# AegisIK/DistMLIP

Measured on NVIDIA H100. Metric: atoms/sec (energy+forces) CHGNet a-Si r_cut=5A, higher is better.
Workload: dtype f32

## Files before the change

### distmlip_b200/csrc/engine.cu

```cuda
#include <dlfcn.h>
#include <nccl.h>

#include <cmath>
#include <condition_variable>
#include <mutex>
#include <thread>
#include <cstring>
#include <map>
#include <new>
#include <set>
#include <string>
#include <vector>

#include <algorithm>
#include <array>

#include "atomic_virial.cuh"
#include "graph.cuh"
#include "kernels.cuh"
#include "mace_state.cuh"
#include "tn_state.cuh"

namespace b2m {

// ... 207 lines not shown
  for (int n = 0; n < N; n++)
    for (int k = 0; k < K; k++) {
      const size_t off = ((size_t)(k / 4) * (N / 8) + n / 8) * 32 + (n % 8) * 4 + (k % 4);
      const float x = raw[(size_t)n * K + k];
      const float h = tf32_hi_host(x);
      o[off] = h;
      o[(size_t)N * Kpad + off] = x - h;
    }
  return o;
}

static std::vector<float> permute_k8(const std::vector<float>& raw, int N, int K) {
  std::vector<float> o(raw.size());
  for (int n = 0; n < N; n++)
    for (int k = 0; k < K; k++) {
      const int q = k % 8;
      o[(size_t)n * K + k] = raw[(size_t)n * K + (k - q) + (q < 4 ? 2 * q : 2 * (q - 4) + 1)];
    }
  return o;
}

static std::vector<float> second_layer_can(const std::vector<float>& raw128x64, bool transposed) {
  std::vector<float> out;
  for (int br = 0; br < 2; br++) {
    std::vector<float> blk(raw128x64.begin() + (size_t)br * 4096, raw128x64.begin() + (size_t)(br + 1) * 4096);
    if (transposed) blk = transpose(blk, 64, 64);
    const auto c = canon_split(permute_k8(blk, 64, 64), 64, 64, 64);
    out.insert(out.end(), c.begin(), c.end());
  }
  return out;
}
static std::vector<float> line_reverse_can(const std::vector<float>& raw128x64) {
  return canon_split(permute_k8(transpose(raw128x64, 128, 64), 64, 128), 64, 128, 128);
}
static std::vector<float> radial_can(const std::vector<float>& M, const std::vector<float>& Wab) {
  auto k8 = [](const std::vector<float>& w, int row0) {
    std::vector<float> o(64 * 8);
    for (int n = 0; n < 64; n++)
      for (int k = 0; k < 8; k++) o[(size_t)n * 8 + k] = w[(size_t)(row0 + n) * NR + k];
    return canon_split(permute_k8(o, 64, 8), 64, 8, 8);
  };
  std::vector<float> out;
  for (const auto& c : {k8(M, 0), k8(M, 64), k8(Wab, 0)}) out.insert(out.end(), c.begin(), c.end());
  for (int j = 0; j < 128; j++) out.push_back(M[(size_t)j * NR + 8]);
  for (int c = 0; c < 64; c++) out.push_back(Wab[(size_t)c * NR + 8]);
  B2M_REQUIRE(out.size() == ATOM_RAD, B2M_ERR_INVALID, "atom-conv radial block size");
  return out;
}

static TcW pack_tc(Packer& P, const std::vector<float>& W, int K, int N, int kmax = 128) {
  TcW w;
  w.K = K, w.N = N;
  for (int k0 = 0; k0 < K;) {
    const int kc = K - k0 >= kmax ? kmax : 64;
    for (int n0 = 0; n0 < N;) {
      const int nc = kc == 64 && N - n0 >= 128 ? 128 : 64;
      std::vector<float> raw((size_t)nc * kc);
      for (int n = 0; n < nc; n++)
        for (int k = 0; k < kc; k++) raw[(size_t)n * kc + k] = W[(size_t)(k0 + k) * N + n0 + n];
      w.blk.push_back({k0, kc, n0, nc, P.add(canon_split(raw, nc, kc, kc))});
      n0 += nc;
    }
    k0 += kc;
  }
  return w;
}
static void pack_tc2(Packer& P, const std::vector<float>& W, int K, int N, TcW& fwd, TcW& rev, int rev_kmax = 128) {
  fwd = pack_tc(P, W, K, N);
  rev = pack_tc(P, transpose(W, K, N), N, K, rev_kmax);
}
static void tc_mm(b2m_engine* e, const float* A, int lda, const TcW& W, float* out, int ldc, int M, bool accum,
                  const float* bias = nullptr, const float* R = nullptr, int ldr = 0, int epi = 0, float* Cpre = nullptr,
                  const float* Pre = nullptr, int ldp = 0) {
  B2M_REQUIRE(epi != 1 || W.blk.back().k0 == 0, B2M_ERR_INVALID, "row GEMM: SiLU epilogue over several K chunks");
  for (const TcW::Blk& b : W.blk) {
    const bool first = b.k0 == 0, last = b.k0 + b.kc == W.K;
    launch_gemm_wg(e->st, A + b.k0, lda, e->wbuf.p + b.off, out + b.n0, ldc, M, b.nc, b.kc,
                   first && bias ? bias + b.n0 : nullptr, first && R ? R + b.n0 : nullptr, ldr, accum || !first,
                   epi == 2 && !last ? 0 : epi, Cpre ? Cpre + b.n0 : nullptr, epi == 2 && last ? Pre + b.n0 : nullptr,
                   ldp, e->num_sms);
  }
}

static void finalize_weights(b2m_engine* e) {
  const int nb = e->desc.n_blocks;
  for (auto& kv : e->host_w) {
    const std::string& k = kv.first;
    bool bad = k.find("atom_graph_layers") != std::string::npos &&
               (k.find("edge_update_func") != std::string::npos || k.find("weight_func") != std::string::npos);
    bad = bad || (k.find("bond_graph_layers") != std::string::npos && k.find("weight_func") != std::string::npos);
    bad = bad || k.find("state_embedding") != std::string::npos || k.find("normalization") != std::string::npos;
    B2M_REQUIRE(!bad, B2M_ERR_INVALID,
                "unsupported CHGNet option (bond_update_hidden_dims / layer_bond_weights / state / norm): " + k);
  }
  e->consumed.clear();
  Packer P;
  std::map<std::string, size_t> off;
  auto put = [&](const std::string& name, const std::vector<float>& v) { off[name] = P.add(v); };
  auto linear = [&](const std::vector<float>& w, int out, int in, TcW& fwd, TcW& rev) {
    pack_tc2(P, transpose(w, out, in), in, out, fwd, rev);
  };

  const auto& f2 = W(e, "bond_expansion.frequencies", {NR});
  const auto& f3 = W(e, "threebody_bond_expansion.frequencies", {NR});
  const auto& fa = W(e, "angle_expansion.frequencies", {5});
  for (int k = 0; k < NR; k++) {
    e->rp2.freq[k] = f2[k];
    e->rp3.freq[k] = f3[k];
  }
  e->rp2.rc = (float)e->desc.cutoff;
  e->rp3.rc = (float)e->desc.three_body_cutoff;
  e->rp2.norm = (float)std::sqrt(2.0 / e->desc.cutoff);
  e->rp3.norm = (float)std::sqrt(2.0 / e->desc.three_body_cutoff);
  e->rp2.p = e->rp3.p = e->desc.cutoff_exponent;
  put("fa", fa);
  put("emb", W(e, "atom_embedding.weight", {e->desc.n_elem, D}));
  const auto& Wbe = W(e, "bond_embedding.layers.0.weight", {D, NR});
  put("Wbe", Wbe);
  put("Wae", W(e, "angle_embedding.layers.0.weight", {D, NF}));
  const auto& Wabw = W(e, "atom_bond_weights.weight", {D, NR});
  put("W3bw", W(e, "threebody_bond_weights.weight", {D, NR}));

  e->aw.resize(nb);
  for (int l = 0; l < nb; l++) {
    const std::string p = "atom_graph_layers." + std::to_string(l) + ".conv_layer.";
    const auto W1 = vcat(W(e, p + "node_update_func.layers.layers.0.weight", {D, 3 * D}),
                         W(e, p + "node_update_func.gates.layers.0.weight", {D, 3 * D}));
    const auto b1 = vcat(W(e, p + "node_update_func.layers.layers.0.bias", {D}),
                         W(e, p + "node_update_func.gates.layers.0.bias", {D}));
    const auto W1s = cols(W1, 128, 192, 0), W1e = cols(W1, 128, 192, 64), W1t = cols(W1, 128, 192, 128);
    const auto W2 = vcat(W(e, p + "node_update_func.layers.layers.1.weight", {D, D}),
                         W(e, p + "node_update_func.gates.layers.1.weight", {D, D}));
    const auto b2 = vcat(W(e, p + "node_update_func.layers.layers.1.bias", {D}),
                         W(e, p + "node_update_func.gates.layers.1.bias", {D}));
    const auto& Wout = W(e, p + "node_out_func.weight", {D, D});
    std::vector<float> M(128 * 9);
    for (int j = 0; j < 128; j++)
      for (int k = 0; k < 9; k++) {
        double s = 0;
        for (int c = 0; c < 64; c++) s += (double)W1e[(size_t)j * 64 + c] * (double)Wbe[(size_t)c * 9 + k];
        M[j * 9 + k] = (float)s;
      }
    const std::string q = "a" + std::to_string(l) + ".";
    AtomLayerW& w = e->aw[l];
    linear(W1s, 128, 64, w.W1s, w.W1sT);
    linear(W1e, 128, 64, w.W1e, w.W1eT);
    linear(W1t, 128, 64, w.W1t, w.W1tT);
    linear(Wout, 64, 64, w.Wout, w.WoutT);
    put(q + "b1", b1);
    put(q + "radial", radial_can(M, Wabw));
    put(q + "W2can", second_layer_can(W2, false));
    put(q + "W2Tcan", second_layer_can(W2, true));
    put(q + "b2", b2);
  }
  e->bw.resize(nb - 1);
  for (int l = 0; l < nb - 1; l++) {
    const std::string p = "bond_graph_layers." + std::to_string(l) + ".conv_layer.";
    const auto W1 = vcat(W(e, p + "node_update_func.layers.layers.0.weight", {D, 4 * D}),
                         W(e, p + "node_update_func.gates.layers.0.weight", {D, 4 * D}));
    const auto b1 = vcat(W(e, p + "node_update_func.layers.layers.0.bias", {D}),
                         W(e, p + "node_update_func.gates.layers.0.bias", {D}));
    const auto W1a = cols(W1, 128, 256, 0), W1g = cols(W1, 128, 256, 64), W1c = cols(W1, 128, 256, 128),
               W1b = cols(W1, 128, 256, 192);
    const auto W2 = vcat(W(e, p + "node_update_func.layers.layers.1.weight", {D, D}),
                         W(e, p + "node_update_func.gates.layers.1.weight", {D, D}));
    const auto b2 = vcat(W(e, p + "node_update_func.layers.layers.1.bias", {D}),
// ... 170 lines not shown
  NCCL_CK(g_nccl.GroupEnd());
  B2M_CK(cudaEventRecord(e->ev_halo, e->cst));
}
static void halo_forward_end(b2m_engine* e) {
  if (e->world <= 1 || e->debug_no_halo) return;
  if (e->leader != nullptr) {
    b2m_engine* L = e->leader;
    const int k = e->hpoint++;
    L->gsync.arrive_and_wait();
    for (int q = 0; q < e->world; q++)
      B2M_CK(cudaStreamWaitEvent(e->st, L->parts[q]->hev[k], 0));
    return;
  }
  B2M_CK(cudaStreamWaitEvent(e->st, e->ev_halo, 0));
}
static void halo_backward(b2m_engine* e, float* gbuf, bool bonds, int width = D) {
  if (e->world <= 1 || e->debug_no_halo) return;
  Graph& g = e->g;
  const size_t W = (size_t)width;
  const int* nto = bonds ? g.nb_to : g.n_to;
  const int* toff = bonds ? g.bto_off : g.to_off;
  const int* nfrom = bonds ? g.nb_from : g.n_from;
  const int* foff = bonds ? g.bfrom_off : g.from_off;
  const int* list = bonds ? g.bto_list.p : g.to_list.p;
  const size_t base = bonds ? (size_t)g.B_own : (size_t)g.n_own;
  const size_t nhalo = bonds ? (size_t)g.B_halo : (size_t)g.n_halo;
  if (e->leader != nullptr) {
    b2m_engine* L = e->leader;
    const int k = e->hpoint;
    for (int q = 0; q < e->world; q++) {
      if (q == e->rank || nfrom[q] <= 0) continue;
      b2m_engine* pe = L->parts[q];
      const size_t ptoff = bonds ? (size_t)pe->g.bto_off[e->rank] : (size_t)pe->g.to_off[e->rank];
      B2M_CK(cudaMemcpyAsync(pe->precv[k & 1].p + ptoff * W, gbuf + (base + foff[q]) * W, (size_t)nfrom[q] * W * sizeof(float),
                             cudaMemcpyDefault, e->st));
    }
    launch_zero_rows(e->st, gbuf + base * W, nhalo * W);
    cudaEvent_t ev = next_halo_event(e);
    B2M_CK(cudaEventRecord(ev, e->st));
    e->hpoint++;
    L->gsync.arrive_and_wait();
    for (int q = 0; q < e->world; q++)
      if (q != e->rank) B2M_CK(cudaStreamWaitEvent(e->st, L->parts[q]->hev[k], 0));
    for (int q = 0; q < e->world; q++)
      if (q != e->rank && nto[q] > 0)
        launch_scatter_add_rows(e->st, nto[q], (int)W, list + toff[q], e->precv[k & 1].p + (size_t)toff[q] * W, gbuf);
    return;
  }
  NCCL_CK(g_nccl.GroupStart());
  for (int q = 0; q < e->world; q++) {
    if (q == e->rank) continue;
    if (nfrom[q] > 0)
      NCCL_CK(g_nccl.Send(gbuf + (base + foff[q]) * W, (size_t)nfrom[q] * W, ncclFloat32, q, e->comm, e->st));
    if (nto[q] > 0)
      NCCL_CK(g_nccl.Recv(e->recvbuf.p + (size_t)toff[q] * W, (size_t)nto[q] * W, ncclFloat32, q, e->comm, e->st));
  }
  NCCL_CK(g_nccl.GroupEnd());
  for (int q = 0; q < e->world; q++)
    if (nto[q] > 0)
      launch_scatter_add_rows(e->st, nto[q], (int)W, list + toff[q], e->recvbuf.p + (size_t)toff[q] * W, gbuf);
  launch_zero_rows(e->st, gbuf + base * W, nhalo * W);
}

#include "engine_tn.inl"
#include "engine_mace.inl"

static AtomConvArgs atom_args(b2m_engine* e, int l) {
  Graph& g = e->g;
  const AtomLayerW& w = e->aw[l];
  AtomConvArgs a;
  memset(&a, 0, sizeof a);
  a.E = g.E;
  a.e_src = g.e_src.p, a.e_dst = g.e_dst.p, a.e_bond = g.e_bond.p, a.e_vec = g.e_vec.p;
  const int ps = e->proj_slot(l);
  a.Aproj = e->ApL[ps].p, a.Cproj = e->CpL[ps].p, a.Qproj = l > 0 ? e->QpL[ps].p : nullptr;
  a.radial = w.radial, a.W2can = w.W2can, a.W2Tcan = w.W2Tcan, a.b2 = w.b2;
  a.rp = e->rp2;
  return a;
}
static void atom_projections(b2m_engine* e, int l) {
  Graph& g = e->g;
  const AtomLayerW& w = e->aw[l];
  const int ps = e->proj_slot(l);
  tc_mm(e, e->x[l].p, D, w.W1s, e->ApL[ps].p, D2, g.n_loc, false);
  tc_mm(e, e->x[l].p, D, w.W1t, e->CpL[ps].p, D2, g.n_own, false, w.b1);
  if (l > 0) tc_mm(e, e->h[l].p, D, w.W1e, e->QpL[ps].p, D2, g.B_own, false);
}
static void atom_layer_fwd(b2m_engine* e, int l) {
  Graph& g = e->g;
  const AtomLayerW& w = e->aw[l];
  atom_projections(e, l);
  launch_zero_rows(e->st, e->agg.p, (int64_t)g.n_own * D);
  AtomConvArgs a = atom_args(e, l);
  a.agg = e->agg.p;
  cudaEvent_t e0, e1;
  B2M_CK(cudaEventCreate(&e0));
  B2M_CK(cudaEventCreate(&e1));
  B2M_CK(cudaEventRecord(e0, e->st));
  launch_atomconv_fwd(e->st, a, e->num_sms);
  B2M_CK(cudaEventRecord(e1, e->st));
  e->gather_ev.push_back({e0, e1});
  tc_mm(e, e->agg.p, D, w.Wout, e->x[l + 1].p, D, g.n_own, false, nullptr, e->x[l].p, D);
}
static void atom_layer_bwd(b2m_engine* e, int l) {
  Graph& g = e->g;
  const AtomLayerW& w = e->aw[l];
  tc_mm(e, e->gx.p, D, w.WoutT, e->gagg.p, D, g.n_own, false);
  AtomConvArgs a = atom_args(e, l);
  a.gagg = e->gagg.p;
  a.gd = e->gd.p;
  const bool need_gx = l > 0;
  if (need_gx) {
    launch_zero_rows(e->st, e->gA.p, (int64_t)g.n_loc * D2);
    launch_zero_rows(e->st, e->gC.p, (int64_t)g.n_own * D2);
    a.gA = e->gA.p, a.gC = e->gC.p, a.gQ = e->gQ.p;
  }
  launch_atomconv_bwd(e->st, a, e->num_sms);
  if (need_gx) {
    tc_mm(e, e->gA.p, D2, w.W1sT, e->gx.p, D, g.n_loc, true);
    tc_mm(e, e->gC.p, D2, w.W1tT, e->gx.p, D, g.n_own, true);
    tc_mm(e, e->gQ.p, D2, w.W1eT, e->gh.p, D, g.B_own, true);
  }
}

static LineArgs line_args(b2m_engine* e, int l, bool hidden) {
  Graph& g = e->g;
  const BondLayerW& w = e->bw[l];
  LineArgs a;
  memset(&a, 0, sizeof a);
  a.A = g.A;
  a.a_in = g.a_in.p, a.a_out = g.a_out.p, a.a_ctr = g.a_ctr.p;
  a.ang = e->ang[l].p;
  a.Ha = e->Ha.p, a.Hb = e->Hb.p, a.Xc = e->Xc.p;
  if (hidden) {
    a.Wgcan = w.Wgcan, a.WgTcan = w.WgTcan, a.W2can = w.W2can, a.W2Tcan = w.W2Tcan, a.b2 = w.b2;
  } else {
    a.Wgcan = w.WAgcan, a.WgTcan = w.WAgTcan;
  }
  return a;
}
static void line_proj_Ha(b2m_engine* e, int l, bool hidden) {
  const BondLayerW& w = e->bw[l];
  const float* hsrc = hidden ? e->h[l].p : e->h[l + 1].p;
  tc_mm(e, hsrc, D, hidden ? w.W1a : w.WAa, e->Ha.p, D2, e->g.B_loc, false);
}
static void line_proj_Hb(b2m_engine* e, int l, bool hidden) {
  const BondLayerW& w = e->bw[l];
  const float* hsrc = hidden ? e->h[l].p : e->h[l + 1].p;
  tc_mm(e, hsrc, D, hidden ? w.W1b : w.WAb, e->Hb.p, D2, e->g.B_own, false, hidden ? w.b1 : w.bA);
}
static void line_proj_Xc(b2m_engine* e, int l, bool hidden) {
  const BondLayerW& w = e->bw[l];
  tc_mm(e, e->x[l + 1].p, D, hidden ? w.W1c : w.WAc, e->Xc.p, D2, e->g.n_loc, false);
}
static void line_projections(b2m_engine* e, int l, bool hidden) {
  line_proj_Ha(e, l, hidden), line_proj_Hb(e, l, hidden), line_proj_Xc(e, l, hidden);
}
static void line_bwd_common(b2m_engine* e, int l, bool hidden, LineArgs& a) {
  Graph& g = e->g;
  const BondLayerW& w = e->bw[l];
  launch_zero_rows(e->st, e->gHa.p, (int64_t)g.B_loc * D2);
  launch_zero_rows(e->st, e->gHb.p, (int64_t)g.B_own * D2);
  launch_zero_rows(e->st, e->gXc.p, (int64_t)g.n_loc * D2);
  a.gang = e->gang.p, a.gHa = e->gHa.p, a.gHb = e->gHb.p, a.gXc = e->gXc.p;
  launch_line_bwd(e->st, a, hidden, e->num_sms);
  tc_mm(e, e->gHa.p, D2, hidden ? w.W1aT : w.WAaT, e->gh.p, D, g.B_loc, true);
  tc_mm(e, e->gHb.p, D2, hidden ? w.W1bT : w.WAbT, e->gh.p, D, g.B_own, true);
  tc_mm(e, e->gXc.p, D2, hidden ? w.W1cT : w.WAcT, e->gx.p, D, g.n_loc, true);
}

static void forward(b2m_engine* e) {
  Graph& g = e->g;
  const int nb = e->desc.n_blocks;
  launch_embed(e->st, g.n_loc, g.type.p, e->d_emb, e->x[0].p);
  launch_bond_init(e->st, g.B_loc, g.b_vec.p, e->rp2, e->d_Wbe, e->h[0].p);
  launch_angle_init(e->st, g.A, g.a_in.p, g.a_out.p, g.b_vec.p, e->d_fa, e->d_Wae, e->ang[0].p);
  for (int l = 0; l < nb - 1; l++) {
    atom_layer_fwd(e, l);
    const BondLayerW& w = e->bw[l];
    halo_forward_begin(e, false, l + 1);
    line_proj_Ha(e, l, true), line_proj_Hb(e, l, true);
    halo_forward_end(e);
    line_proj_Xc(e, l, true);
    launch_zero_rows(e->st, e->aggB.p, (int64_t)g.B_own * D);
    LineArgs a = line_args(e, l, true);
    a.aggB = e->aggB.p;
    launch_line_fwd(e->st, a, true, e->num_sms);
    tc_mm(e, e->aggB.p, D, w.Wout, e->upd[l].p, D, g.B_own, false);
    launch_bond_update_fwd(e->st, g.B_own, g.b_vec.p, e->rp3, e->d_W3bw, e->h[l].p, e->upd[l].p, e->h[l + 1].p);
    if (l < nb - 2) {
      halo_forward_begin(e, true, l + 1);
      line_proj_Hb(e, l, false), line_proj_Xc(e, l, false);
      halo_forward_end(e);
      line_proj_Ha(e, l, false);
      LineArgs b = line_args(e, l, false);
      b.ang_out = e->ang[l + 1].p;
      launch_line_fwd(e->st, b, false, e->num_sms);
    }
  }
  launch_rowdot(e->st, g.n_own, e->x[nb - 1].p, e->d_Ws, e->bs, e->site.p, nullptr, nullptr, nullptr, 1.f);
  atom_layer_fwd(e, nb - 1);
  tc_mm(e, e->x[nb].p, D, e->F0, e->y1p.p, D, g.n_own, false, e->d_c0);
  launch_silu(e->st, (int64_t)g.n_own * D, e->y1p.p, e->y1.p);
  tc_mm(e, e->y1.p, D, e->F1, e->y2p.p, D, g.n_own, false, e->d_c1);
  launch_silu(e->st, (int64_t)g.n_own * D, e->y2p.p, e->y2.p);
  B2M_CK(cudaMemsetAsync(e->scal.p, 0, 16 * sizeof(double), e->st));
  launch_rowdot(e->st, g.n_own, e->y2.p, e->d_F2, e->c2, e->e_atom.p, e->scal.p, g.type.p, e->d_eref,
                (float)e->desc.data_std, g.gid.p, e->atomic ? e->atom_e.p : nullptr, e->desc.data_mean / cell_atoms(e),
                e->hf_n ? e->hf_w.p : nullptr);
}

static void backward(b2m_engine* e) {
  Graph& g = e->g;
  const int nb = e->desc.n_blocks;
  launch_zero_rows(e->st, e->gd.p, g.E);
  launch_zero_rows(e->st, e->gdb.p, g.B_loc);
  launch_zero_rows(e->st, e->gbvec.p, (int64_t)g.B_loc * 3);
  launch_zero_rows(e->st, e->gh.p, (int64_t)g.B_loc * D);
  launch_zero_rows(e->st, e->gang.p, (g.A + 127) / 128 * 128 * D);
  launch_zero_rows(e->st, e->gx.p, (int64_t)g.n_loc * D);
  launch_zero_rows(e->st, e->forces.p, g.N * 3);
  launch_readout_seed(e->st, g.n_own, e->y2p.p, e->d_F2, (float)e->desc.data_std, e->gy2.p, g.gid.p,
                      e->hf_n ? e->hf_w.p : nullptr);
  tc_mm(e, e->gy2.p, D, e->F1T, e->gy1.p, D, g.n_own, false);
  launch_dsilu_mul(e->st, (int64_t)g.n_own * D, e->y1p.p, e->gy1.p);
  tc_mm(e, e->gy1.p, D, e->F0T, e->gx.p, D, g.n_own, false);
  atom_layer_bwd(e, nb - 1);
  for (int l = nb - 2; l >= 0; l--) {
    const BondLayerW& w = e->bw[l];
    if (l < nb - 2) {
      line_projections(e, l, false);
      LineArgs a = line_args(e, l, false);
      line_bwd_common(e, l, false, a);
      halo_backward(e, e->gh.p, true);
    }
    launch_bond_update_bwd(e->st, g.B_own, g.b_vec.p, e->rp3, e->d_W3bw, e->gh.p, e->upd[l].p, e->gupd.p, e->gdb.p);
    tc_mm(e, e->gupd.p, D, w.WoutT, e->gaggB.p, D, g.B_own, false);
    line_projections(e, l, true);
    LineArgs a = line_args(e, l, true);
    a.gaggB = e->gaggB.p;
    line_bwd_common(e, l, true, a);
    halo_backward(e, e->gx.p, false);
    atom_layer_bwd(e, l);
  }
  launch_h0_bwd(e->st, g.B_loc, g.b_vec.p, e->rp2, e->d_Wbe, e->gh.p, e->gdb.p);
  launch_angle_init_bwd(e->st, g.A, g.a_in.p, g.a_out.p, g.b_vec.p, e->d_fa, e->d_Wae, e->gang.p, e->gbvec.p);
  float* avir = e->atomic ? e->atom_vir.p : nullptr;
  launch_edge_final(e->st, g.E, g.e_src.p, g.e_dst.p, g.e_bond.p, g.e_vec.p, g.gid.p, e->gd.p, e->gdb.p, e->gbvec.p,
                    e->forces.p, e->scal.p + 1, avir);
  launch_halo_bond_final(e->st, g.B_own, g.B_loc, g.b_src_gid.p, g.b_dst.p, g.b_vec.p, g.gid.p, e->gdb.p, e->gbvec.p,
                         e->forces.p, e->scal.p + 1, avir);
}

#define LAUNCH_HF(kern, n, st, ...)                              \
  do {                                                           \
    if ((n) > 0) {                                               \
      kern<<<cdiv((n), 256), 256, 0, st>>>(__VA_ARGS__);         \
      B2M_CK(cudaGetLastError());                                \
      g_launch_count++;                                          \
    }                                                            \
  } while (0)

__global__ void k_hf_weights(int64_t N, int64_t n, const double* __restrict__ cart, double cx, double cy, double cz,
                             int alpha, float* __restrict__ w) {
// ... 891 lines not shown
```

### distmlip_b200/csrc/kernels.cuh

```cuda
#pragma once
#include "common.cuh"

namespace b2m {

constexpr int TM = 128;
constexpr int LDA = 68;
constexpr int NT = 256;

struct RadialParams {
  float freq[NR];
  float rc;
  float norm;
  int p;
};

void launch_embed(cudaStream_t st, int n, const int* type, const float* emb, float* x0);
void launch_bond_init(cudaStream_t st, int nb, const float4* b_vec, RadialParams rp, const float* W ,
                      float* out );
void launch_angle_init(cudaStream_t st, int64_t na, const int* a_in, const int* a_out, const float4* b_vec,
                       const float* fa , const float* Wae , float* ang0 );
void launch_silu(cudaStream_t st, int64_t n, const float* pre, float* out);
void launch_dsilu_mul(cudaStream_t st, int64_t n, const float* pre, float* g);
void launch_zero_rows(cudaStream_t st, float* p, int64_t nfloats);

constexpr int ATOM_RAD_M = 0, ATOM_RAD_WAB = 2048, ATOM_RAD_M8 = 3072, ATOM_RAD_WAB8 = 3200, ATOM_RAD = 3264;
struct AtomConvArgs {
  int64_t E;
  const int* e_src;
  const int* e_dst;
  const int* e_bond;
  const float4* e_vec;
  const float* Aproj;
  const float* Cproj;
  const float* Qproj;
  const float* radial;
  const float* W2can;
  const float* W2Tcan;
  const float* b2;
  RadialParams rp;
  float* agg;
  const float* gagg;
  float* gA;
  float* gC;
  float* gQ;
  float* gd;
};
void launch_atomconv_fwd(cudaStream_t st, const AtomConvArgs& a, int num_sms);
void launch_atomconv_bwd(cudaStream_t st, const AtomConvArgs& a, int num_sms);

struct LineArgs {
  int64_t A;
  const int* a_in;
  const int* a_out;
  const int* a_ctr;
  const float* ang;
  const float* Ha;
  const float* Hb;
  const float* Xc;
  const float* Wgcan;
  const float* WgTcan;
  const float* W2can;
  const float* W2Tcan;
  const float* b2;
  float* aggB;
  float* ang_out;
  const float* gaggB;
  float* gang;
  float* gHa;
  float* gHb;
  float* gXc;
};
void launch_line_fwd(cudaStream_t st, const LineArgs& a, bool hidden, int num_sms);
void launch_line_bwd(cudaStream_t st, const LineArgs& a, bool hidden, int num_sms);

void launch_bond_update_fwd(cudaStream_t st, int nb, const float4* b_vec, RadialParams rp3, const float* W3bw,
                            const float* h, const float* upd, float* hout);
void launch_bond_update_bwd(cudaStream_t st, int nb, const float4* b_vec, RadialParams rp3, const float* W3bw,
                            const float* gh, const float* upd, float* gupd, float* gdb);
void launch_h0_bwd(cudaStream_t st, int nb, const float4* b_vec, RadialParams rp, const float* Wbe, const float* gh0,
                   float* gdb);
void launch_angle_init_bwd(cudaStream_t st, int64_t na, const int* a_in, const int* a_out, const float4* b_vec,
                           const float* fa, const float* Wae, const float* gang0, float* gbvec);

void launch_rowdot(cudaStream_t st, int n, const float* X, const float* w, float bias, float* out, double* sum,
                   const int* type, const double* elem_ref, float scale, const int* gid = nullptr,
                   double* atom_e = nullptr, double mean_per_atom = 0.0, const float* wgt = nullptr);
void launch_readout_seed(cudaStream_t st, int n, const float* pre, const float* w, float scale, float* g,
                         const int* gid = nullptr, const float* wgt = nullptr);

void launch_edge_final(cudaStream_t st, int64_t E, const int* e_src, const int* e_dst, const int* e_bond,
                       const float4* e_vec, const int* gid, const float* gd, const float* gdb, const float* gbvec,
                       float* forces , double* virial , float* atom_vir = nullptr);
void launch_halo_bond_final(cudaStream_t st, int b0, int b1, const int* b_src_gid, const int* b_dst,
                            const float4* b_vec, const int* gid, const float* gdb, const float* gbvec, float* forces,
                            double* virial, float* atom_vir = nullptr);

void launch_gather_rows(cudaStream_t st, int n, int width, const int* idx, const float* src, float* dst);
void launch_scatter_add_rows(cudaStream_t st, int n, int width, const int* idx, const float* src, float* dst);

}

namespace b2m {
void launch_gemm_wg(cudaStream_t st, const float* A, int lda, const float* Bcan, float* C, int ldc, int M, int N, int K,
                    const float* bias, const float* R, int ldr, bool accum, int epi, float* Cpre, const float* Pre,
                    int ldp, int num_sms);
struct TcW {
  struct Blk {
    int k0, kc, n0, nc;
    size_t off;
  };
  int K = 0, N = 0;
  std::vector<Blk> blk;
};
}

namespace b2m {
struct TnRadial {
  int nr;
  int nrp;
  float width;
  float rc;
  float mu[64];
};
struct TnGemm {
  const float* A = nullptr;
  int lda = 0;
  int64_t zA = 0;
  const float *B0 = nullptr, *B1 = nullptr, *B2 = nullptr;
  int bsel = 0;
  float* C = nullptr;
  int ldc = 0;
  int64_t zC = 0;
  float* Cpre = nullptr;
  const float* Pre = nullptr;
  int ldp = 0;
  const float* bias = nullptr;
  int M = 0, N = 0, K = 0, accum = 0, epi = 0;
};
void launch_tn_gemm(cudaStream_t st, const TnGemm& g, int nz);
void launch_tn_edge_geom(cudaStream_t st, int64_t E, const float4* e_vec, const TnRadial& rp, float* rbf, float* cut);
void launch_tn_embed_agg(cudaStream_t st, int n_own, const int* row_ptr, const int* e_src, const int* type,
                         const float* U, const float* V, const float* P, const float* cut, const float4* e_vec,
                         float* T0, float* nr0);
void launch_tn_layernorm(cudaStream_t st, int rows, int W, const float* x, const float* gamma, const float* beta,
                         float* y, float* stats);
void launch_tn_layernorm_bwd(cudaStream_t st, int rows, int W, const float* x, const float* stats, const float* gamma,
                             const float* gy, float* gx);
void launch_tn_embed_out(cudaStream_t st, int n, const float* T0m, const float* s2p, float* X0);
void launch_tn_embed_out_bwd(cudaStream_t st, int n, const float* T0m, const float* s2p, const float* gX0, float* gT0m,
                             float* gs2p);
void launch_tn_norm_bwd_add(cudaStream_t st, int n, const float* T0, const float* gnr0, float* gT0);
void launch_tn_embed_agg_bwd(cudaStream_t st, int64_t E, const int* e_src, const int* e_dst, const int* type,
                             const float* U, const float* V, const float* P, const float* cut, const float4* e_vec,
                             const float* gT0, float* gP, float* gC, float* gvh);
void launch_tn_scale(cudaStream_t st, int n, const float* X, float* Xh, float* q);
void launch_tn_scale_bwd(cudaStream_t st, int n, const float* X, const float* q, float* g);
void launch_tn_msg(cudaStream_t st, int n_own, const int* row_ptr, const int* e_src, const float* f3p, const float* cut,
                   const float* Y, float* msg);
void launch_tn_msg_bwd(cudaStream_t st, int n_own, const int* row_ptr, const int* e_src, const float* f3p,
                       const float* cut, const float* Y, const float* gmsg, float* g3, float* gC, float* gY);
void launch_tn_prod(cudaStream_t st, int n, const float* msg, const float* Y, int so3, float* Pn);
void launch_tn_prod_bwd(cudaStream_t st, int n, const float* msg, const float* Y, int so3, const float* gPn,
                        float* gmsg, float* gY);
void launch_tn_update(cudaStream_t st, int n, const float* Xh, const float* dX, float* Xn);
void launch_tn_update_bwd(cudaStream_t st, int n, const float* dX, const float* gXn, float* gdX);
void launch_tn_invariants(cudaStream_t st, int n, const float* X, float* inv);
void launch_tn_invariants_bwd(cudaStream_t st, int n, const float* X, const float* ginv, float* gX);
void launch_tn_readout_final(cudaStream_t st, int n, int W, const float* hL, const float* wL, float bL, const float* hG,
                             const float* wG, float bG, const int* type, const double* eref, float scale, float* lout,
                             float* gout, float* e_atom, double* energy, const int* gid = nullptr,
                             double* atom_e = nullptr, double mean_per_atom = 0.0, const float* wgt = nullptr);
void launch_tn_readout_seed(cudaStream_t st, int n, int W, const float* lout, const float* gout, float scale,
                            const float* wL, const float* wG, const float* preL, const float* preG, float* gL,
                            float* gG, const int* gid = nullptr, const float* wgt = nullptr);
void launch_tn_edge_final(cudaStream_t st, int64_t E, const int* e_src, const int* e_dst, const float4* e_vec,
                          const int* gid, const TnRadial& rp, const float* g_rbf, const float* gC, const float* gvh,
                          float* gd, float* forces, double* virial, float* atom_vir = nullptr);
}
```

### distmlip_b200/csrc/kernels_wg.cu

```cuda
#include "kernels.cuh"
#include "wgmma.cuh"

namespace b2m {


template <int K, int N, int EPI>
__global__ void __launch_bounds__(256, 1)
    k_gemm_wg(const float* __restrict__ A, int lda, const float* __restrict__ Bcan, float* __restrict__ C, int ldc, int M,
              const float* __restrict__ bias, const float* __restrict__ R, int ldr, int accum, float* __restrict__ Cpre,
              const float* __restrict__ Pre, int ldp) {
  constexpr int KH = K / 64;
  constexpr int NR = N / 2;
  constexpr uint32_t LBO_B = (N / 8) * 128;
  constexpr uint32_t LBO_A = (128 / 8) * 128;
  constexpr uint32_t A_PLANE = 128 * 64 * 4;
  extern __shared__ __align__(1024) float smem[];
  float* Bs = smem;
  float* As = smem + 2 * N * K;
  const int tid = threadIdx.x, wg = tid >> 7, wt = tid & 127;
  const int warp = wt >> 5, lane = tid & 31;
  const int ntiles = (M + 127) / 128;

  float4 pre[8];
  auto load_chunk = [&](int t, int kh) {
#pragma unroll
    for (int i = 0; i < 8; i++) {
      const int f = tid + 256 * i;
      const int row = t * 128 + (f >> 7) * 8 + (f & 7);
      pre[i] = make_float4(0.f, 0.f, 0.f, 0.f);
      if (row < M) pre[i] = *reinterpret_cast<const float4*>(A + (size_t)row * lda + kh * 64 + ((f >> 3) & 15) * 4);
    }
  };
  if ((int)blockIdx.x < ntiles) load_chunk(blockIdx.x, 0);
  for (int i = tid; i < 2 * N * K / 4; i += 256) reinterpret_cast<float4*>(Bs)[i] = reinterpret_cast<const float4*>(Bcan)[i];
  const uint32_t a_addr = s_u32(As) + (uint32_t)wg * 1024u, b_addr = s_u32(Bs);

  float d[NR];
  for (int t = blockIdx.x; t < ntiles; t += gridDim.x) {
    const int row0 = t * 128;
#pragma unroll 1
    for (int kh = 0; kh < KH; kh++) {
      __syncthreads();
#pragma unroll
      for (int i = 0; i < 8; i++) {
        const int f = tid + 256 * i;
        const int off = (((f >> 3) & 15) * 16 + (f >> 7)) * 32 + (f & 7) * 4;
        const float xv[4] = {pre[i].x, pre[i].y, pre[i].z, pre[i].w};
        uint32_t h[4], l[4];
#pragma unroll
        for (int j = 0; j < 4; j++) {
          h[j] = tf32_hi_bits(xv[j]);
          l[j] = __float_as_uint(xv[j] - __uint_as_float(h[j]));
        }
        *reinterpret_cast<uint4*>(As + off) = make_uint4(h[0], h[1], h[2], h[3]);
        *reinterpret_cast<uint4*>(As + 128 * 64 + off) = make_uint4(l[0], l[1], l[2], l[3]);
      }
      fence_proxy_async_smem();
      __syncthreads();
      if (kh + 1 < KH)
        load_chunk(t, kh + 1);
      else if (t + (int)gridDim.x < ntiles)
        load_chunk(t + gridDim.x, 0);
      acc_fence(d);
      wgmma_fence();
#pragma unroll
      for (int term = 0; term < 3; term++) {
        const uint32_t asel = a_addr + (term == 1 ? A_PLANE : 0u);
        const uint32_t bsel = b_addr + (term == 2 ? (uint32_t)(N * K) * 4u : 0u) + (uint32_t)kh * 16u * LBO_B;
#pragma unroll
        for (int ks = 0; ks < 8; ks++) {
          const uint64_t ad = gmma_desc(asel + ks * 2 * LBO_A, LBO_A, 128u);
          const uint64_t bd = gmma_desc(bsel + ks * 2 * LBO_B, LBO_B, 128u);
          const int scale_d = (kh > 0 || term > 0 || ks > 0) ? 1 : 0;
          if constexpr (N == 128)
            wgmma_tf32_n128(d, ad, bd, scale_d);
          else
            wgmma_tf32_n64(d, ad, bd, scale_d);
        }
      }
      wgmma_commit();
      wgmma_wait_all();
      acc_fence(d);
    }
    const int rbase = row0 + wg * 64 + warp * 16 + (lane >> 2);
    const float* addsrc = R ? R : (accum ? C : nullptr);
    const int addld = R ? ldr : ldc;
#pragma unroll
    for (int h = 0; h < 2; h++) {
      const int row = rbase + 8 * h;
      if (row >= M) continue;
#pragma unroll
      for (int j = 0; j < N / 8; j++) {
        const int col = 8 * j + 2 * (lane & 3);
        float2 o = make_float2(d[4 * j + 2 * h], d[4 * j + 2 * h + 1]);
        if (bias) {
          const float2 b = *reinterpret_cast<const float2*>(bias + col);
          o.x += b.x, o.y += b.y;
        }
        if (addsrc) {
          const float2 x = *reinterpret_cast<const float2*>(addsrc + (size_t)row * addld + col);
          o.x += x.x, o.y += x.y;
        }
        float2* cp = reinterpret_cast<float2*>(C + (size_t)row * ldc + col);
        if (R && accum) {
          const float2 c = *cp;
          o.x += c.x, o.y += c.y;
        }
        if constexpr (EPI == 1) {
          *reinterpret_cast<float2*>(Cpre + (size_t)row * ldc + col) = o;
          o = make_float2(silu_(o.x), silu_(o.y));
        } else if constexpr (EPI == 2) {
          const float2 pv = *reinterpret_cast<const float2*>(Pre + (size_t)row * ldp + col);
          o.x *= dsilu_(pv.x), o.y *= dsilu_(pv.y);
        }
        *cp = o;
      }
    }
  }
}

template <int K, int N, int EPI>
static void launch_gemm_wg_t(cudaStream_t st, const float* A, int lda, const float* Bcan, float* C, int ldc, int M,
                             const float* bias, const float* R, int ldr, bool accum, float* Cpre, const float* Pre,
                             int ldp, int num_sms) {
  constexpr size_t bytes = (size_t)(2 * N * K + 2 * 128 * 64) * 4;
  static_assert(bytes <= 232448, "shared memory budget");
  constexpr int per_sm = bytes <= 232448 / 2 - 1024 ? 2 : 1;
  static PerDeviceOnce attr;
  if (auto once_ = attr.first(); once_)
    B2M_CK(cudaFuncSetAttribute(k_gemm_wg<K, N, EPI>, cudaFuncAttributeMaxDynamicSharedMemorySize, (int)bytes));
  auto al = [](const void* p, uintptr_t n) { return p == nullptr || (((uintptr_t)p) & (n - 1)) == 0; };
  B2M_REQUIRE(lda % 4 == 0 && ldc % 2 == 0 && (R == nullptr || ldr % 2 == 0) && (Pre == nullptr || ldp % 2 == 0) &&
                  al(A, 16) && al(Bcan, 16) && al(C, 8) && al(bias, 8) && al(R, 8) && al(Cpre, 8) && al(Pre, 8),
              B2M_ERR_INVALID, "gemm_wg operand alignment");
  const int ntiles = (M + 127) / 128;
  const int grid = std::min(ntiles, per_sm * num_sms);
  k_gemm_wg<K, N, EPI><<<grid, 256, bytes, st>>>(A, lda, Bcan, C, ldc, M, bias, R, ldr, accum ? 1 : 0, Cpre, Pre, ldp);
  B2M_CK(cudaGetLastError());
  g_launch_count++;
}

template <int EPI>
static void launch_gemm_wg_s(cudaStream_t st, const float* A, int lda, const float* Bcan, float* C, int ldc, int M, int N,
                             int K, const float* bias, const float* R, int ldr, bool accum, float* Cpre, const float* Pre,
                             int ldp, int num_sms) {
  if (K == 64 && N == 128)
    launch_gemm_wg_t<64, 128, EPI>(st, A, lda, Bcan, C, ldc, M, bias, R, ldr, accum, Cpre, Pre, ldp, num_sms);
  else if (K == 64 && N == 64)
    launch_gemm_wg_t<64, 64, EPI>(st, A, lda, Bcan, C, ldc, M, bias, R, ldr, accum, Cpre, Pre, ldp, num_sms);
  else if (K == 128 && N == 64)
    launch_gemm_wg_t<128, 64, EPI>(st, A, lda, Bcan, C, ldc, M, bias, R, ldr, accum, Cpre, Pre, ldp, num_sms);
  else
    throw Error(B2M_ERR_INVALID, "gemm_wg shape");
}

void launch_gemm_wg(cudaStream_t st, const float* A, int lda, const float* Bcan, float* C, int ldc, int M, int N, int K,
                    const float* bias, const float* R, int ldr, bool accum, int epi, float* Cpre, const float* Pre,
                    int ldp, int num_sms) {
  if (M <= 0) return;
  B2M_REQUIRE(epi == 1 ? Cpre != nullptr : (epi == 2 ? Pre != nullptr : epi == 0), B2M_ERR_INVALID, "gemm_wg epilogue");
  if (epi == 1)
    launch_gemm_wg_s<1>(st, A, lda, Bcan, C, ldc, M, N, K, bias, R, ldr, accum, Cpre, Pre, ldp, num_sms);
  else if (epi == 2)
    launch_gemm_wg_s<2>(st, A, lda, Bcan, C, ldc, M, N, K, bias, R, ldr, accum, Cpre, Pre, ldp, num_sms);
  else
    launch_gemm_wg_s<0>(st, A, lda, Bcan, C, ldc, M, N, K, bias, R, ldr, accum, Cpre, Pre, ldp, num_sms);
}

}
```

Measured before the change: 2.249 million.

## Fuse paired projection GEMMs into single merged tensor-core launches

Adds two merged variants of the wgmma GEMM kernel. The first computes two outputs from the same A tile using two weight images held in shared memory, and is used for the W1s/W1t and Ha/Hb projections. The second concatenates two A operands along K into one accumulation, and is used for the backward gx and gh updates. This cuts kernel launches, repeated reads of A, and read-modify-write passes over the output, at the cost of more shared memory per block and longer per-tile work.

```diff
diff --git a/distmlip_b200/csrc/engine.cu b/distmlip_b200/csrc/engine.cu
--- a/distmlip_b200/csrc/engine.cu
+++ b/distmlip_b200/csrc/engine.cu
@@ -313,6 +313,21 @@
   }
 }
 
+static void tc_mm_pair(b2m_engine* e, const float* A, int lda, const TcW& W1, float* out1, int M1, const float* b1,
+                       const TcW& W2, float* out2, int M2, const float* b2, int ldc) {
+  B2M_REQUIRE(W1.blk.size() == 1 && W2.blk.size() == 1 && W1.K == 64 && W1.N == 128 && W2.K == 64 && W2.N == 128,
+              B2M_ERR_INVALID, "row GEMM pair: one 64 x 128 block each");
+  launch_gemm_wg_pair(e->st, A, lda, M1, e->wbuf.p + W1.blk[0].off, out1, ldc, b1, e->wbuf.p + W2.blk[0].off, out2, ldc,
+                      b2, M2, e->num_sms);
+}
+static void tc_mm_acc2(b2m_engine* e, const float* A1, const TcW& W1, int M1, const float* A2, const TcW& W2, int M2,
+                       int lda, float* out, int ldc) {
+  B2M_REQUIRE(W1.blk.size() == 1 && W2.blk.size() == 1 && W1.K == 128 && W1.N == 64 && W2.K == 128 && W2.N == 64,
+              B2M_ERR_INVALID, "row GEMM accumulate pair: one 128 x 64 block each");
+  launch_gemm_wg_acc2(e->st, A1, lda, M1, A2, lda, M2, e->wbuf.p + W1.blk[0].off, e->wbuf.p + W2.blk[0].off, out, ldc,
+                      true, e->num_sms);
+}
+
 static void finalize_weights(b2m_engine* e) {
   const int nb = e->desc.n_blocks;
   for (auto& kv : e->host_w) {
@@ -649,8 +664,7 @@
   Graph& g = e->g;
   const AtomLayerW& w = e->aw[l];
   const int ps = e->proj_slot(l);
-  tc_mm(e, e->x[l].p, D, w.W1s, e->ApL[ps].p, D2, g.n_loc, false);
-  tc_mm(e, e->x[l].p, D, w.W1t, e->CpL[ps].p, D2, g.n_own, false, w.b1);
+  tc_mm_pair(e, e->x[l].p, D, w.W1s, e->ApL[ps].p, g.n_loc, nullptr, w.W1t, e->CpL[ps].p, g.n_own, w.b1, D2);
   if (l > 0) tc_mm(e, e->h[l].p, D, w.W1e, e->QpL[ps].p, D2, g.B_own, false);
 }
 static void atom_layer_fwd(b2m_engine* e, int l) {
@@ -684,8 +698,7 @@
   }
   launch_atomconv_bwd(e->st, a, e->num_sms);
   if (need_gx) {
-    tc_mm(e, e->gA.p, D2, w.W1sT, e->gx.p, D, g.n_loc, true);
-    tc_mm(e, e->gC.p, D2, w.W1tT, e->gx.p, D, g.n_own, true);
+    tc_mm_acc2(e, e->gA.p, w.W1sT, g.n_loc, e->gC.p, w.W1tT, g.n_own, D2, e->gx.p, D);
     tc_mm(e, e->gQ.p, D2, w.W1eT, e->gh.p, D, g.B_own, true);
   }
 }
@@ -720,8 +733,14 @@
   const BondLayerW& w = e->bw[l];
   tc_mm(e, e->x[l + 1].p, D, hidden ? w.W1c : w.WAc, e->Xc.p, D2, e->g.n_loc, false);
 }
+static void line_proj_HaHb(b2m_engine* e, int l, bool hidden) {
+  const BondLayerW& w = e->bw[l];
+  const float* hsrc = hidden ? e->h[l].p : e->h[l + 1].p;
+  tc_mm_pair(e, hsrc, D, hidden ? w.W1a : w.WAa, e->Ha.p, e->g.B_loc, nullptr, hidden ? w.W1b : w.WAb, e->Hb.p,
+             e->g.B_own, hidden ? w.b1 : w.bA, D2);
+}
 static void line_projections(b2m_engine* e, int l, bool hidden) {
-  line_proj_Ha(e, l, hidden), line_proj_Hb(e, l, hidden), line_proj_Xc(e, l, hidden);
+  line_proj_HaHb(e, l, hidden), line_proj_Xc(e, l, hidden);
 }
 static void line_bwd_common(b2m_engine* e, int l, bool hidden, LineArgs& a) {
   Graph& g = e->g;
@@ -731,8 +750,7 @@
   launch_zero_rows(e->st, e->gXc.p, (int64_t)g.n_loc * D2);
   a.gang = e->gang.p, a.gHa = e->gHa.p, a.gHb = e->gHb.p, a.gXc = e->gXc.p;
   launch_line_bwd(e->st, a, hidden, e->num_sms);
-  tc_mm(e, e->gHa.p, D2, hidden ? w.W1aT : w.WAaT, e->gh.p, D, g.B_loc, true);
-  tc_mm(e, e->gHb.p, D2, hidden ? w.W1bT : w.WAbT, e->gh.p, D, g.B_own, true);
+  tc_mm_acc2(e, e->gHa.p, hidden ? w.W1aT : w.WAaT, g.B_loc, e->gHb.p, hidden ? w.W1bT : w.WAbT, g.B_own, D2, e->gh.p, D);
   tc_mm(e, e->gXc.p, D2, hidden ? w.W1cT : w.WAcT, e->gx.p, D, g.n_loc, true);
 }
 
@@ -746,7 +764,7 @@
     atom_layer_fwd(e, l);
     const BondLayerW& w = e->bw[l];
     halo_forward_begin(e, false, l + 1);
-    line_proj_Ha(e, l, true), line_proj_Hb(e, l, true);
+    line_proj_HaHb(e, l, true);
     halo_forward_end(e);
     line_proj_Xc(e, l, true);
     launch_zero_rows(e->st, e->aggB.p, (int64_t)g.B_own * D);
diff --git a/distmlip_b200/csrc/kernels.cuh b/distmlip_b200/csrc/kernels.cuh
--- a/distmlip_b200/csrc/kernels.cuh
+++ b/distmlip_b200/csrc/kernels.cuh
@@ -104,6 +104,11 @@
 void launch_gemm_wg(cudaStream_t st, const float* A, int lda, const float* Bcan, float* C, int ldc, int M, int N, int K,
                     const float* bias, const float* R, int ldr, bool accum, int epi, float* Cpre, const float* Pre,
                     int ldp, int num_sms);
+void launch_gemm_wg_pair(cudaStream_t st, const float* A, int lda, int M, const float* B1, float* C1, int ldc1,
+                         const float* bias1, const float* B2, float* C2, int ldc2, const float* bias2, int M2,
+                         int num_sms);
+void launch_gemm_wg_acc2(cudaStream_t st, const float* A1, int lda1, int M, const float* A2, int lda2, int M2,
+                         const float* B1, const float* B2, float* C, int ldc, bool accum, int num_sms);
 struct TcW {
   struct Blk {
     int k0, kc, n0, nc;
diff --git a/distmlip_b200/csrc/kernels_wg.cu b/distmlip_b200/csrc/kernels_wg.cu
--- a/distmlip_b200/csrc/kernels_wg.cu
+++ b/distmlip_b200/csrc/kernels_wg.cu
@@ -3,37 +3,131 @@
 
 namespace b2m {
 
-
-template <int K, int N, int EPI>
+struct WgSecond {
+  const float* A2;
+  int lda2;
+  int M2;
+  const float* B2;
+  float* C2;
+  int ldc2;
+  const float* bias2;
+};
+
+template <int K, int N, int EPI, int MERGE>
 __global__ void __launch_bounds__(256, 1)
     k_gemm_wg(const float* __restrict__ A, int lda, const float* __restrict__ Bcan, float* __restrict__ C, int ldc, int M,
               const float* __restrict__ bias, const float* __restrict__ R, int ldr, int accum, float* __restrict__ Cpre,
-              const float* __restrict__ Pre, int ldp) {
-  constexpr int KH = K / 64;
+              const float* __restrict__ Pre, int ldp, const WgSecond sec) {
+  constexpr int KO = K / 64;
+  constexpr int KH = (MERGE == 2 ? 2 : 1) * KO;
+  constexpr int IMG = 2 * N * K;
   constexpr int NR = N / 2;
   constexpr uint32_t LBO_B = (N / 8) * 128;
   constexpr uint32_t LBO_A = (128 / 8) * 128;
   constexpr uint32_t A_PLANE = 128 * 64 * 4;
   extern __shared__ __align__(1024) float smem[];
   float* Bs = smem;
-  float* As = smem + 2 * N * K;
+  float* As = smem + (MERGE ? 2 : 1) * IMG;
   const int tid = threadIdx.x, wg = tid >> 7, wt = tid & 127;
   const int warp = wt >> 5, lane = tid & 31;
   const int ntiles = (M + 127) / 128;
 
   float4 pre[8];
   auto load_chunk = [&](int t, int kh) {
+    const bool second = MERGE == 2 && kh >= KO;
+    const float* src = second ? sec.A2 : A;
+    const int ld = second ? sec.lda2 : lda, mrows = second ? sec.M2 : M, kc = second ? kh - KO : kh;
 #pragma unroll
     for (int i = 0; i < 8; i++) {
       const int f = tid + 256 * i;
       const int row = t * 128 + (f >> 7) * 8 + (f & 7);
       pre[i] = make_float4(0.f, 0.f, 0.f, 0.f);
-      if (row < M) pre[i] = *reinterpret_cast<const float4*>(A + (size_t)row * lda + kh * 64 + ((f >> 3) & 15) * 4);
+      if (row < mrows) pre[i] = *reinterpret_cast<const float4*>(src + (size_t)row * ld + kc * 64 + ((f >> 3) & 15) * 4);
     }
   };
   if ((int)blockIdx.x < ntiles) load_chunk(blockIdx.x, 0);
-  for (int i = tid; i < 2 * N * K / 4; i += 256) reinterpret_cast<float4*>(Bs)[i] = reinterpret_cast<const float4*>(Bcan)[i];
+  for (int i = tid; i < IMG / 4; i += 256) reinterpret_cast<float4*>(Bs)[i] = reinterpret_cast<const float4*>(Bcan)[i];
+  if constexpr (MERGE != 0)
+    for (int i = tid; i < IMG / 4; i += 256)
+      reinterpret_cast<float4*>(Bs + IMG)[i] = reinterpret_cast<const float4*>(sec.B2)[i];
   const uint32_t a_addr = s_u32(As) + (uint32_t)wg * 1024u, b_addr = s_u32(Bs);
+  const int rbase0 = wg * 64 + warp * 16 + (lane >> 2);
+
+  auto mma_chunk = [&](float (&d)[NR], uint32_t wblk, int kc, bool accumulate) {
+    acc_fence(d);
+    wgmma_fence();
+#pragma unroll
+    for (int term = 0; term < 3; term++) {
+      const uint32_t asel = a_addr + (term == 1 ? A_PLANE : 0u);
+      const uint32_t bsel = wblk + (term == 2 ? (uint32_t)(N * K) * 4u : 0u) + (uint32_t)kc * 16u * LBO_B;
+#pragma unroll
+      for (int ks = 0; ks < 8; ks++) {
+        const uint64_t ad = gmma_desc(asel + ks * 2 * LBO_A, LBO_A, 128u);
+        const uint64_t bd = gmma_desc(bsel + ks * 2 * LBO_B, LBO_B, 128u);
+        const int scale_d = (accumulate || term > 0 || ks > 0) ? 1 : 0;
+        if constexpr (N == 128)
+          wgmma_tf32_n128(d, ad, bd, scale_d);
+        else
+          wgmma_tf32_n64(d, ad, bd, scale_d);
+      }
+    }
+    wgmma_commit();
+    wgmma_wait_all();
+    acc_fence(d);
+  };
+  auto epilogue2 = [&](const float (&d)[NR], int row0) {
+#pragma unroll
+    for (int h = 0; h < 2; h++) {
+      const int row = row0 + rbase0 + 8 * h;
+      if (row >= sec.M2) continue;
+#pragma unroll
+      for (int j = 0; j < N / 8; j++) {
+        const int col = 8 * j + 2 * (lane & 3);
+        float2 o = make_float2(d[4 * j + 2 * h], d[4 * j + 2 * h + 1]);
+        if (sec.bias2) {
+          const float2 b = *reinterpret_cast<const float2*>(sec.bias2 + col);
+          o.x += b.x, o.y += b.y;
+        }
+        *reinterpret_cast<float2*>(sec.C2 + (size_t)row * sec.ldc2 + col) = o;
+      }
+    }
+  };
+  auto epilogue = [&](const float (&d)[NR], int row0) {
+    const int rbase = row0 + rbase0;
+    const float* addsrc = R ? R : (accum ? C : nullptr);
+    const int addld = R ? ldr : ldc;
+#pragma unroll
+    for (int h = 0; h < 2; h++) {
+      const int row = rbase + 8 * h;
+      if (row >= M) continue;
+#pragma unroll
+      for (int j = 0; j < N / 8; j++) {
+        const int col = 8 * j + 2 * (lane & 3);
+        float2 o = make_float2(d[4 * j + 2 * h], d[4 * j + 2 * h + 1]);
+        if (bias) {
+          const float2 b = *reinterpret_cast<const float2*>(bias + col);
+          o.x += b.x, o.y += b.y;
+        }
+        if (addsrc) {
+          const float2 x = *reinterpret_cast<const float2*>(addsrc + (size_t)row * addld + col);
+          o.x += x.x, o.y += x.y;
+        }
+        float2* cp = reinterpret_cast<float2*>(C + (size_t)row * ldc + col);
+        if (R && accum) {
+          const float2 c = *cp;
+          o.x += c.x, o.y += c.y;
+        }
+        if constexpr (EPI == 1) {
+          *reinterpret_cast<float2*>(Cpre + (size_t)row * ldc + col) = o;
+          o = make_float2(silu_(o.x), silu_(o.y));
+        } else if constexpr (EPI == 2) {
+          const float2 pv = *reinterpret_cast<const float2*>(Pre + (size_t)row * ldp + col);
+          o.x *= dsilu_(pv.x), o.y *= dsilu_(pv.y);
+        }
+        *cp = o;
+      }
+    }
+  };
 
   float d[NR];
   for (int t = blockIdx.x; t < ntiles; t += gridDim.x) {
@@ -61,81 +155,39 @@
         load_chunk(t, kh + 1);
       else if (t + (int)gridDim.x < ntiles)
         load_chunk(t + gridDim.x, 0);
-      acc_fence(d);
-      wgmma_fence();
-#pragma unroll
-      for (int term = 0; term < 3; term++) {
-        const uint32_t asel = a_addr + (term == 1 ? A_PLANE : 0u);
-        const uint32_t bsel = b_addr + (term == 2 ? (uint32_t)(N * K) * 4u : 0u) + (uint32_t)kh * 16u * LBO_B;
-#pragma unroll
-        for (int ks = 0; ks < 8; ks++) {
-          const uint64_t ad = gmma_desc(asel + ks * 2 * LBO_A, LBO_A, 128u);
-          const uint64_t bd = gmma_desc(bsel + ks * 2 * LBO_B, LBO_B, 128u);
-          const int scale_d = (kh > 0 || term > 0 || ks > 0) ? 1 : 0;
-          if constexpr (N == 128)
-            wgmma_tf32_n128(d, ad, bd, scale_d);
-          else
-            wgmma_tf32_n64(d, ad, bd, scale_d);
-        }
-      }
-      wgmma_commit();
-      wgmma_wait_all();
-      acc_fence(d);
-    }
-    const int rbase = row0 + wg * 64 + warp * 16 + (lane >> 2);
-    const float* addsrc = R ? R : (accum ? C : nullptr);
-    const int addld = R ? ldr : ldc;
-#pragma unroll
-    for (int h = 0; h < 2; h++) {
-      const int row = rbase + 8 * h;
-      if (row >= M) continue;
-#pragma unroll
-      for (int j = 0; j < N / 8; j++) {
-        const int col = 8 * j + 2 * (lane & 3);
-        float2 o = make_float2(d[4 * j + 2 * h], d[4 * j + 2 * h + 1]);
-        if (bias) {
-          const float2 b = *reinterpret_cast<const float2*>(bias + col);
-          o.x += b.x, o.y += b.y;
-        }
-        if (addsrc) {
-          const float2 x = *reinterpret_cast<const float2*>(addsrc + (size_t)row * addld + col);
-          o.x += x.x, o.y += x.y;
-        }
-        float2* cp = reinterpret_cast<float2*>(C + (size_t)row * ldc + col);
-        if (R && accum) {
-          const float2 c = *cp;
-          o.x += c.x, o.y += c.y;
-        }
-        if constexpr (EPI == 1) {
-          *reinterpret_cast<float2*>(Cpre + (size_t)row * ldc + col) = o;
-          o = make_float2(silu_(o.x), silu_(o.y));
-        } else if constexpr (EPI == 2) {
-          const float2 pv = *reinterpret_cast<const float2*>(Pre + (size_t)row * ldp + col);
-          o.x *= dsilu_(pv.x), o.y *= dsilu_(pv.y);
-        }
-        *cp = o;
+      mma_chunk(d, b_addr + (MERGE == 2 && kh >= KO ? (uint32_t)IMG * 4u : 0u), MERGE == 2 ? kh % KO : kh, kh > 0);
+    }
+    epilogue(d, row0);
+    if constexpr (MERGE == 1) {
+      if (row0 < sec.M2) {
+        mma_chunk(d, b_addr + (uint32_t)IMG * 4u, 0, false);
+        epilogue2(d, row0);
       }
     }
   }
 }
 
-template <int K, int N, int EPI>
+template <int K, int N, int EPI, int MERGE = 0>
 static void launch_gemm_wg_t(cudaStream_t st, const float* A, int lda, const float* Bcan, float* C, int ldc, int M,
                              const float* bias, const float* R, int ldr, bool accum, float* Cpre, const float* Pre,
-                             int ldp, int num_sms) {
-  constexpr size_t bytes = (size_t)(2 * N * K + 2 * 128 * 64) * 4;
+                             int ldp, int num_sms, const WgSecond& sec = WgSecond{}) {
+  static_assert(MERGE == 0 || EPI == 0, "merged launches have plain epilogues");
+  constexpr size_t bytes = (size_t)((MERGE ? 2 : 1) * 2 * N * K + 2 * 128 * 64) * 4;
   static_assert(bytes <= 232448, "shared memory budget");
   constexpr int per_sm = bytes <= 232448 / 2 - 1024 ? 2 : 1;
   static PerDeviceOnce attr;
   if (auto once_ = attr.first(); once_)
-    B2M_CK(cudaFuncSetAttribute(k_gemm_wg<K, N, EPI>, cudaFuncAttributeMaxDynamicSharedMemorySize, (int)bytes));
+    B2M_CK(cudaFuncSetAttribute(k_gemm_wg<K, N, EPI, MERGE>, cudaFuncAttributeMaxDynamicSharedMemorySize, (int)bytes));
   auto al = [](const void* p, uintptr_t n) { return p == nullptr || (((uintptr_t)p) & (n - 1)) == 0; };
   B2M_REQUIRE(lda % 4 == 0 && ldc % 2 == 0 && (R == nullptr || ldr % 2 == 0) && (Pre == nullptr || ldp % 2 == 0) &&
-                  al(A, 16) && al(Bcan, 16) && al(C, 8) && al(bias, 8) && al(R, 8) && al(Cpre, 8) && al(Pre, 8),
+                  al(A, 16) && al(Bcan, 16) && al(C, 8) && al(bias, 8) && al(R, 8) && al(Cpre, 8) && al(Pre, 8) &&
+                  (sec.A2 == nullptr || sec.lda2 % 4 == 0) && (sec.C2 == nullptr || sec.ldc2 % 2 == 0) &&
+                  al(sec.A2, 16) && al(sec.B2, 16) && al(sec.C2, 8) && al(sec.bias2, 8),
               B2M_ERR_INVALID, "gemm_wg operand alignment");
   const int ntiles = (M + 127) / 128;
   const int grid = std::min(ntiles, per_sm * num_sms);
-  k_gemm_wg<K, N, EPI><<<grid, 256, bytes, st>>>(A, lda, Bcan, C, ldc, M, bias, R, ldr, accum ? 1 : 0, Cpre, Pre, ldp);
+  k_gemm_wg<K, N, EPI, MERGE>
+      <<<grid, 256, bytes, st>>>(A, lda, Bcan, C, ldc, M, bias, R, ldr, accum ? 1 : 0, Cpre, Pre, ldp, sec);
   B2M_CK(cudaGetLastError());
   g_launch_count++;
 }
@@ -167,4 +219,23 @@
     launch_gemm_wg_s<0>(st, A, lda, Bcan, C, ldc, M, N, K, bias, R, ldr, accum, Cpre, Pre, ldp, num_sms);
 }
 
-}
+void launch_gemm_wg_pair(cudaStream_t st, const float* A, int lda, int M, const float* B1, float* C1, int ldc1,
+                         const float* bias1, const float* B2, float* C2, int ldc2, const float* bias2, int M2,
+                         int num_sms) {
+  if (M <= 0) return;
+  B2M_REQUIRE(M2 >= 0 && M2 <= M && B2 != nullptr && C2 != nullptr, B2M_ERR_INVALID, "gemm_wg pair operands");
+  const WgSecond sec{nullptr, 0, M2, B2, C2, ldc2, bias2};
+  launch_gemm_wg_t<64, 128, 0, 1>(st, A, lda, B1, C1, ldc1, M, bias1, nullptr, 0, false, nullptr, nullptr, 0, num_sms,
+                                  sec);
+}
+
+void launch_gemm_wg_acc2(cudaStream_t st, const float* A1, int lda1, int M, const float* A2, int lda2, int M2,
+                         const float* B1, const float* B2, float* C, int ldc, bool accum, int num_sms) {
+  if (M <= 0) return;
+  B2M_REQUIRE(M2 >= 0 && M2 <= M && A2 != nullptr && B2 != nullptr, B2M_ERR_INVALID, "gemm_wg accumulate pair operands");
+  const WgSecond sec{A2, lda2, M2, B2, nullptr, 0, nullptr};
+  launch_gemm_wg_t<128, 64, 0, 2>(st, A1, lda1, B1, C, ldc, M, nullptr, nullptr, 0, accum, nullptr, nullptr, 0, num_sms,
+                                  sec);
+}
+
+}
```

After: 2.269 million (median of 6 runs). About the same (+0.9%).
